# 34j/vr180-convert

Hardware: NVIDIA B200
Metric: SBS equirect output Mpix/s (higher is better)
Workload: dtype f64 coordinates / u8 fixed-point (INTER_BITS=5) sampling

## Files before the change

vr180-convert_b200/csrc/tiled.cu:

```cuda
#include "tiled.cuh"

namespace vr180 {
namespace tiled {

struct TileGeom {
    int rsel;
    int bx0, ry0;
    int x0, y0;
};

template <class M, int NV, bool DYN, int FR, bool SPLIT = false, bool VPAIR = false>
__device__ __forceinline__ void frame_loop(const RemapArgs& a, const TmaMaps& tm, int v_begin, int f0, int f1,
                                           const typename M::Pixel (&pc)[M::kPx], const TileGeom& tg, const int pitch,
                                           uint8_t* smem, int band, int cg, const DynRadius& dr,
                                           const double (&nx)[M::kPx], const double (&ny)[M::kPx], const short* tab) {
    static_assert(FR == 1 || !DYN, "a per-frame radius gives every frame its own rectangle");
    static_assert(M::kOutTiles / FR >= 2, "at least two out buffers of one item each");
    constexpr int kOutTileBytes = M::kTileH * kTileW * 3;
    constexpr int kOutItemBytes = FR * kOutTileBytes;
    constexpr int OB = M::kOutTiles / FR < kOutBufs ? M::kOutTiles / FR : kOutBufs;
    const int tid = threadIdx.x, lane = tid & 31, warp = tid >> 5;
    uint32_t s_stage = smem_u32(smem);
    asm volatile("" : "+r"(s_stage));
    const uint32_t s_full = s_stage + Lay<M>::kOffBar;
    const uint32_t s_ofull = s_full + 2 * kMaxStages * 8, s_oempty = s_ofull + kOutBufs * 8, s_out = s_stage + Lay<M>::kOffOut;

    int2* const s_org = reinterpret_cast<int2*>(smem + Lay<M>::kOffOrg);
    static_assert(!VPAIR || (SPLIT && FR == 2 && NV == 2 && !DYN), "an eye pair is two one-frame boxes of two views");
    const int n_items = VPAIR ? (f1 - f0) : ((f1 - f0 + FR - 1) / FR) * NV;
    const int rect_bytes = (M::kRowsMin + tg.rsel * kRowsStep) * pitch;
    const int stage_bytes = FR * rect_bytes;
    const int frame_pitch = SPLIT ? (rect_bytes + 127) & ~127 : rect_bytes;
    const int stage_stride = (FR * frame_pitch + 127) & ~127;
    static_assert(Lay<M>::kStageArea % 128 == 0 && Lay<M>::kStageArea / 128 <= 1024, "float quotient below");
    const int S = min(kMaxStages, (int)__fdividef((float)(Lay<M>::kStageArea / 128) + 0.5f, (float)(stage_stride >> 7)));

    if (warp == kSamplers / 32) {
        if (lane != 0) return;
        const CUtensorMap* const map0 = &tm.src[v_begin][(pitch - kPitchMin) / kPitchStep][tg.rsel];
        const int dst_x0 = (a.view[v_begin].dst_x_offset + tg.x0) * 3;
        const int dst_x1 = (a.view[v_begin + NV - 1].dst_x_offset + tg.x0) * 3;
        int p_item = 0, p_stage = 0;
        auto load = [&]() {
            const uint32_t bar = s_full + p_stage * 8;
            const int v = (NV == 2 && !VPAIR) ? (p_item & 1) : 0;
            const int f = VPAIR ? f0 + p_item : f0 + FR * ((NV == 2) ? (p_item >> 1) : p_item);
            int bx0 = tg.bx0, ry0 = tg.ry0;
            if (DYN) {
                const double rad = __ldg(dr.radius + f);
                if (rad == rad) {
                    int xlo, xhi, ylo, yhi;
                    dyn_range<M>(dr.ext[0], dr.ext[1], rad, dr.cx, xlo, xhi);
                    dyn_range<M>(dr.ext[2], dr.ext[3], rad, dr.cy, ylo, yhi);
                    const TileRect rc = tile_rect<M>(xlo, xhi, ylo, yhi);
                    bx0 = rc.bx0;
                    ry0 = rc.ry0;
                } else {
                    bx0 = ry0 = -(1 << 20);
                }
                s_org[p_stage] = make_int2(bx0, ry0);
            }
            mbar_expect_tx(bar, (uint32_t)stage_bytes);
            if (SPLIT) {
#pragma unroll
                for (int fr = 0; fr < FR; ++fr)
                    tma_load_3d(s_stage + p_stage * stage_stride + fr * frame_pitch,
                                map0 + (VPAIR ? fr : v) * (kWidths * kRowSizes), bx0, ry0, VPAIR ? f : f + fr, bar);
            } else {
                tma_load_3d(s_stage + p_stage * stage_stride, map0 + v * (kWidths * kRowSizes), bx0, ry0, f, bar);
            }
            ++p_item;
            if (++p_stage == S) p_stage = 0;
        };
        for (int n = 0; n < S && n < n_items; ++n) load();
        for (int n = 0; n < n_items; ++n) {
            const int o = n & (OB - 1);
            const int v = (NV == 2 && !VPAIR) ? (n & 1) : 0;
            const int f = VPAIR ? f0 + n : f0 + FR * ((NV == 2) ? (n >> 1) : n);
            mbar_wait(s_ofull + o * 8, (uint32_t)(n / OB) & 1u);
            if (n + S < n_items) load();
            if (SPLIT) {
#pragma unroll
                for (int fr = 0; fr < FR; ++fr)
                    tma_store_3d(&tm.dst, (VPAIR ? fr : v) ? dst_x1 : dst_x0, tg.y0, VPAIR ? f : f + fr,
                                 s_out + o * kOutItemBytes + fr * kOutTileBytes);
            } else {
                tma_store_3d(&tm.dst, v ? dst_x1 : dst_x0, tg.y0, f, s_out + o * kOutItemBytes);
            }
            bulk_commit();
            bulk_wait_read<0>();
            mbar_arrive(s_oempty + o * 8);
        }
        bulk_wait_read<0>();
        return;
    }

    const int sub = lane & 3;
    const uint32_t out_sel = sub == 0 ? 0x4210u : (sub == 1 ? 0x5421u : 0x6542u);
    const bool writer = sub != 3;
    constexpr int kOutStep = M::kRowPatch ? kTileW * 3 : 24;
    const int sw = band * (4 / M::kPx) + cg;
    uint32_t outp = s_out + (M::kRowPatch ? (M::kPx * sw) * (kTileW * 3) + (3 * (lane >> 2) + sub) * 4
                                          : (4 * band + (lane >> 3)) * (kTileW * 3) + M::kPx * cg * 24 +
                                                (3 * ((lane & 7) >> 2) + sub) * 4);
    uint32_t flags = (writer ? 1u : 0u) | (lane == 0 ? 2u : 0u);
    asm volatile("" : "+r"(outp), "+r"(flags));

    int st = 0;
    uint32_t ph = 0;
    typename M::Pixel cur[M::kPx];
    double cur_rad = CUDART_NAN;
    bool cur_have = false;
#pragma unroll
    for (int k = 0; k < M::kPx; ++k) cur[k] = pc[k];
    for (int n = 0; n < n_items; ++n) {
        mbar_wait(s_full + st * 8, ph);
        const uint32_t buf = s_stage + st * stage_stride;
        uint32_t res[FR][M::kPx];
        if (DYN) {
            const int f = f0 + ((NV == 2) ? (n >> 1) : n);
            const double rad = __ldg(dr.radius + f);
            if (!(rad == cur_rad)) {
                const int2 org = s_org[st];
                cur_have = rad == rad;
#pragma unroll
                for (int k = 0; k < M::kPx; ++k) {
                    const int qx = denorm_q<M>(nx[k], rad, dr.cx), qy = denorm_q<M>(ny[k], rad, dr.cy);
                    const int off = ((qy >> M::kShift) - M::kLo - org.y) * pitch + 3 * ((qx >> M::kShift) - M::kLo) - org.x;
                    M::set_offset(cur[k], off, cur_have);
                    M::weights(cur[k], qx & 31, qy & 31, tab);
                }
                cur_rad = rad;
            }
#pragma unroll
            for (int k = 0; k < M::kPx; ++k) {
                const uint32_t r = M::sample(buf, cur[k], (uint32_t)pitch);
                res[0][k] = cur_have ? r : 0u;
            }
        }
        uint32_t word[FR][M::kPx];
        if (!DYN && M::kInterp == VR180_INTER_LANCZOS4) {
#pragma unroll
            for (int k = 0; k < M::kPx; ++k) {
                uint32_t r[FR];
                sample_item<M, FR>(buf, (uint32_t)frame_pitch, pc[k], (uint32_t)pitch, r);
#pragma unroll
                for (int fr = 0; fr < FR; ++fr) res[fr][k] = r[fr];
            }
        }
#pragma unroll
        for (int fr = 0; fr < FR; ++fr) {
            if (!DYN && M::kInterp != VR180_INTER_LANCZOS4) {
#pragma unroll
                for (int k = 0; k < M::kPx; ++k) res[fr][k] = M::sample(buf + fr * frame_pitch, pc[k], (uint32_t)pitch);
            }
#pragma unroll
            for (int k = 0; k < M::kPx; ++k)
                word[fr][k] = __byte_perm(res[fr][k], __shfl_down_sync(0xffffffffu, res[fr][k], 1), out_sel);
        }
        const int o = n & (OB - 1);
        if (n >= OB) mbar_wait(s_oempty + o * 8, (uint32_t)(n / OB + 1) & 1u);
        if (flags & 1u) {
            const uint32_t ob = outp + o * kOutItemBytes;
#pragma unroll
            for (int fr = 0; fr < FR; ++fr)
#pragma unroll
                for (int k = 0; k < M::kPx; ++k) sts32(ob + fr * kOutTileBytes + k * kOutStep, word[fr][k]);
        }
        fence_proxy_async();
        __syncwarp();
        if (flags & 2u) mbar_arrive(s_ofull + o * 8);
        if (++st == S) { st = 0; ph ^= 1u; }
    }
}

template <class M, bool DYN, int FR>
__global__ void __launch_bounds__(kThreads, 4)
k_warp_tiled(const __grid_constant__ RemapArgs a, const __grid_constant__ vr180_chain_t chain0,
             const __grid_constant__ vr180_chain_t chain1, const __grid_constant__ TiledParams tp,
             const __grid_constant__ TmaMaps tm) {
    constexpr int kPx = M::kPx;
    constexpr int kChainUnroll = (FR == 1 && !DYN) ? kPx : 1;
    constexpr int kWarpsPerBand = 4 / kPx;
    extern __shared__ __align__(1024) uint8_t smem[];
    double* s_trig = reinterpret_cast<double*>(smem + Lay<M>::kOffTrig);
    int4* s_red = reinterpret_cast<int4*>(smem + Lay<M>::kOffRed);

    const int tid = threadIdx.x, lane = tid & 31, warp = tid >> 5;
    if (tid < 2 * kMaxStages + 2 * kOutBufs) {
        const uint32_t bars = smem_u32(smem + Lay<M>::kOffBar);
        const bool by_warps = (tid >= kMaxStages && tid < 2 * kMaxStages + kOutBufs);
        mbar_init(bars + tid * 8, by_warps ? kSamplers / 32 : 1);
        asm volatile("fence.mbarrier_init.release.cluster;" ::: "memory");
    }
    int* const s_cost = reinterpret_cast<int*>(smem + Lay<M>::kOffCost);
    if (tid < kPitchCands) s_cost[tid] = 0;
    const int tx = blockIdx.x, ty = blockIdx.y, tile = ty * tp.tiles_x + tx;
    const int x0 = tx * kTileW, y0 = ty * M::kTileH;
    const bool two_groups = !a.share_map && a.n_views == 2;
    const int g = two_groups ? (int)(blockIdx.z & 1u) : 0;
    const int chunk = two_groups ? (int)(blockIdx.z >> 1) : (int)blockIdx.z;
    const ViewArgs& mv = a.view[g];
    const int v_begin = g, v_end = a.share_map ? a.n_views : g + 1, nv = v_end - v_begin;
    const int f0 = chunk * a.frames_per_cta, f1 = min(a.n_frames, f0 + a.frames_per_cta);
    const bool sampler = warp < kSamplers / 32;
    const int sw = warp & (kSamplers / 32 - 1), band = sw / kWarpsPerBand, cg = sw % kWarpsPerBand;
    const int lx = M::kRowPatch ? lane : 8 * kPx * cg + (lane & 7), ly = M::kRowPatch ? kPx * sw : 4 * band + (lane >> 3);
    auto pcol = [&](int k) { return M::kRowPatch ? lx : lx + 8 * k; };
    auto prow = [&](int k) { return M::kRowPatch ? ly + k : ly; };
    const bool full_tile = (x0 + kTileW <= a.W) && (y0 + M::kTileH <= a.H);

    TileHdr hdr = {0, 0, 0, 0, 0};
    if (mv.map_kind != VR180_MAPSRC_ANALYTIC && mv.packed) hdr = decode_header(packed_header_raw(mv.packed, tile));
    const bool packed_tile = (hdr.flags & 1) != 0;

    int sx[kPx], sy[kPx];
    double nx[kPx], ny[kPx];
#pragma unroll
    for (int k = 0; k < kPx; ++k) {
        sx[k] = sy[k] = 0;
        nx[k] = ny[k] = 0.0;
    }
    constexpr bool dyn = DYN;
    if (mv.map_kind == VR180_MAPSRC_ANALYTIC) {
        const vr180_chain_t& ch = mv.chain_idx ? chain1 : chain0;
        const StdChain& sc = tp.std[mv.chain_idx ? 1 : 0];
        const bool fastc = sc.valid && sc.fast && !(tp.debug & 256);
        if (sc.valid || tp.sep_prefix) {
            if (tid < 64) {
                const bool is_row = tid >= 32;
                const int idx = tid & 31;
                const double* nm = ch.ops[0].p;
                const double c = (double)((is_row ? y0 : x0) + idx);
                const double n = mul_rn(__ddiv_rn(add_rn(c, -(is_row ? nm[1] : nm[0])), nm[2]), 2.0);
                double sv, cv;
                sincos(mul_rn(n, kHalfPi), &sv, &cv);
                if (fastc) {
                    std_tables(sc.R, sc.lat_is_y != 0, is_row, sv, cv, s_trig, s_trig + 128, idx);
                } else {
                    s_trig[(is_row ? 64 : 0) + idx] = sv;
                    s_trig[(is_row ? 96 : 32) + idx] = cv;
                }
            }
            __syncthreads();
            const bool lat_is_y = ch.ops[1].iparam != 0;
            auto seed = [&](int k, ChainState& s) {
                const double s_row = s_trig[64 + prow(k)], c_row = s_trig[96 + prow(k)];
                const double s_col = s_trig[pcol(k)], c_col = s_trig[32 + pcol(k)];
                s.mode = MODE_VEC3;
                s.x = s.y = s.r = s.ux = s.uy = 0.0;
                if (lat_is_y) {
                    s.vx = mul_rn(c_row, s_col);
                    s.vy = s_row;
                    s.vz = mul_rn(c_row, c_col);
                } else {
                    s.vx = s_col;
                    s.vy = mul_rn(c_col, s_row);
                    s.vz = mul_rn(c_col, c_row);
                }
            };
            if (!sampler) {
            } else if (fastc) {
                auto std_eval = [&](const StdChain& c) {
                    const bool x_fixed = M::kRowPatch ? !c.lat_is_y : (c.lat_is_y != 0);
                    const int fi = M::kRowPatch ? lx : ly;
                    const double* const ft = s_trig + (x_fixed ? 0 : 128) + fi;
                    const double f0 = ft[0], f1 = ft[32], f2 = ft[64], f3 = x_fixed ? ft[96] : 0.0;
#pragma unroll(kChainUnroll)
                    for (int k = 0; k < kPx; ++k) {
                        const int vi = M::kRowPatch ? prow(k) : pcol(k);
                        double vx, vy, vz;
                        if (x_fixed) {
                            vx = fma(f0, s_trig[128 + vi], f1); vy = fma(f0, s_trig[160 + vi], f2); vz = fma(f0, s_trig[192 + vi], f3);
                        } else {
                            const double sc_ = s_trig[vi];
                            vx = fma(sc_, f0, s_trig[32 + vi]); vy = fma(sc_, f1, s_trig[64 + vi]); vz = fma(sc_, f2, s_trig[96 + vi]);
                        }
                        double ox, oy;
                        int qx = 0, qy = 0;
                        if (dyn) {
                            std_pixel<true>(vx, vy, vz, c.poly, c.n_poly, c.den, ox, oy);
                        } else {
                            std_pixel<false>(vx, vy, vz, c.poly, c.n_poly, c.den, ox, oy);
                            qx = M::quant(__double2float_rn(ox));
                            qy = M::quant(__double2float_rn(oy));
                        }
#pragma unroll
                        for (int kk = 0; kk < kPx; ++kk)
                            if (kk == k) { sx[kk] = qx; sy[kk] = qy; nx[kk] = ox; ny[kk] = oy; }
                    }
                };
                if (mv.chain_idx) std_eval(tp.std[1]);
                else std_eval(tp.std[0]);
            } else {
#pragma unroll 1
                for (int k = 0; k < kPx; ++k) {
                    ChainState s;
                    seed(k, s);
                    run_ops(ch, 2, ch.n_ops - (dyn ? 1 : 0), s);
                    to_xy(s);
                    const int qx = M::quant(__double2float_rn(s.x)), qy = M::quant(__double2float_rn(s.y));
#pragma unroll
                    for (int kk = 0; kk < kPx; ++kk)
                        if (kk == k) { sx[kk] = qx; sy[kk] = qy; nx[kk] = s.x; ny[kk] = s.y; }
                }
            }
        } else if (sampler) {
#pragma unroll 1
            for (int k = 0; k < kPx; ++k) {
                double xs, ys;
                if (dyn) eval_chain_normalised(ch, x0 + pcol(k), y0 + prow(k), xs, ys);
                else eval_chain(ch, x0 + pcol(k), y0 + prow(k), xs, ys);
                const int qx = M::quant(__double2float_rn(xs)), qy = M::quant(__double2float_rn(ys));
#pragma unroll
                for (int kk = 0; kk < kPx; ++kk)
                    if (kk == k) { sx[kk] = qx; sy[kk] = qy; nx[kk] = xs; ny[kk] = ys; }
            }
        }
    } else if (sampler) {
        bool unpacked = false;
// ... 14 lines not shown
        for (int k = 0; k < kPx; ++k) {
            if (unpacked) break;
            const int i = x0 + pcol(k), j = y0 + prow(k);
            sx[k] = sy[k] = (int)0x80000000;
            if (i < a.W && j < a.H) {
                if (mv.map_kind == VR180_MAPSRC_FLOAT2) {
                    sx[k] = M::quant(__ldg(mv.xmap + (long long)j * mv.map_pitch + i));
                    sy[k] = M::quant(__ldg(mv.ymap + (long long)j * mv.map_pitch + i));
                } else {
                    const int2 q = __ldg(mv.fixed + (long long)j * mv.map_pitch + i);
                    sx[k] = q.x;
                    sy[k] = q.y;
                }
            }
        }
    }

    bool dynr = dyn;
    if (dyn) {
        const vr180_chain_t& ch = mv.chain_idx ? chain1 : chain0;
        const double r0 = __ldg(mv.radius_dev + f0);
        int same = r0 == r0;
        for (int f = f0 + 1 + lane; f < f1; f += 32) same &= __ldg(mv.radius_dev + f) == r0;
        if (__all_sync(0xffffffffu, same)) {
            dynr = false;
            const double cx = ch.ops[ch.n_ops - 1].p[2], cy = ch.ops[ch.n_ops - 1].p[3];
#pragma unroll
            for (int k = 0; k < kPx; ++k) {
                sx[k] = denorm_q<M>(nx[k], r0, cx);
                sy[k] = denorm_q<M>(ny[k], r0, cy);
            }
        }
    }

    if (!packed_tile) block_box_store<M>(sx, sy, s_red, warp, lane == 0 && sampler);
    DynRadius dr;
    dr.radius = nullptr;
    dr.cx = dr.cy = 0.0;
    dr.ext[0] = dr.ext[1] = dr.ext[2] = dr.ext[3] = 0.0;
    int nan_px = 0;
    if (dynr) {
        double* s_ext = reinterpret_cast<double*>(smem + Lay<M>::kOffExt);
        double e0 = CUDART_INF, e1 = -CUDART_INF, e2 = CUDART_INF, e3 = -CUDART_INF;
        if (sampler) {
#pragma unroll
            for (int k = 0; k < kPx; ++k) {
                nan_px |= (nx[k] != nx[k]) | (ny[k] != ny[k]);
                e0 = fmin(e0, nx[k]);
                e1 = fmax(e1, nx[k]);
                e2 = fmin(e2, ny[k]);
                e3 = fmax(e3, ny[k]);
            }
        }
#pragma unroll
        for (int d = 16; d > 0; d >>= 1) {
            e0 = fmin(e0, __shfl_xor_sync(0xffffffffu, e0, d));
            e1 = fmax(e1, __shfl_xor_sync(0xffffffffu, e1, d));
            e2 = fmin(e2, __shfl_xor_sync(0xffffffffu, e2, d));
            e3 = fmax(e3, __shfl_xor_sync(0xffffffffu, e3, d));
        }
        if (lane == 0 && sampler) {
            s_ext[warp * 4 + 0] = e0;
            s_ext[warp * 4 + 1] = e1;
            s_ext[warp * 4 + 2] = e2;
            s_ext[warp * 4 + 3] = e3;
        }
    }
    nan_px = __syncthreads_or(nan_px);
    static_assert(Lay<M>::kOffRed % 16 == 0, "s_red is read as int4");
    const int4 box = packed_tile ? make_int4(hdr.mnx, hdr.mxx, hdr.mny, hdr.mxy) : block_box_load(s_red, lane);
    const int mnx = box.x, mxx = box.y, mny = box.z, mxy = box.w;
    const TileRect rc = tile_rect<M>(mnx, mxx, mny, mxy);
    const bool vpair = !DYN && FR == 1 && nv == 2;
    const int fr_item = dynr ? 1 : (vpair ? 2 : FR);
    auto stage_fits = [&](int box_rows, int pitch_bytes) {
        const int rect = box_rows * pitch_bytes;
        return ((fr_item * ((DYN || vpair) ? (rect + 127) & ~127 : rect) + 127) & ~127) <= Lay<M>::kStageArea;
    };
    const int src_cols = a.view[v_begin].cols, src_rows = a.view[v_begin].rows;
    auto inside_src = [&](int x_lo, int x_hi, int y_lo, int y_hi) {
        return x_lo - M::kLo >= 0 && x_hi + M::kHi <= src_cols - 1 && y_lo - M::kLo >= 0 && y_hi + M::kHi <= src_rows - 1;
    };
    bool fast = full_tile && rc.wbytes <= kPitchMax && rc.rsel < kRowSizes && mnx > -32768 && mny > -32768 &&
                mxx < 32767 && mxy < 32767 && stage_fits(rc.box_rows, max(rc.wbytes, kPitchMin)) &&
                (tp.zero_border || inside_src(mnx, mxx, mny, mxy));
    int dyn_wbytes = 0, dyn_nrows = 0;
    if (dynr) {
        const double* s_ext = reinterpret_cast<const double*>(smem + Lay<M>::kOffExt);
        dr.ext[0] = dr.ext[2] = CUDART_INF;
        dr.ext[1] = dr.ext[3] = -CUDART_INF;
#pragma unroll
        for (int w = 0; w < kSamplers / 32; ++w) {
            dr.ext[0] = fmin(dr.ext[0], s_ext[w * 4 + 0]);
            dr.ext[1] = fmax(dr.ext[1], s_ext[w * 4 + 1]);
            dr.ext[2] = fmin(dr.ext[2], s_ext[w * 4 + 2]);
            dr.ext[3] = fmax(dr.ext[3], s_ext[w * 4 + 3]);
        }
        const vr180_chain_t& ch = mv.chain_idx ? chain1 : chain0;
        dr.radius = mv.radius_dev;
        dr.cx = ch.ops[ch.n_ops - 1].p[2];
        dr.cy = ch.ops[ch.n_ops - 1].p[3];
        int ok = 1;
        for (int f = f0 + lane; f < f1; f += 32) {
            const double rad = __ldg(dr.radius + f);
            if (rad == rad) {
                int lo, hi, ylo, yhi;
                dyn_range<M>(dr.ext[0], dr.ext[1], rad, dr.cx, lo, hi);
                ok &= (lo > -32768) & (hi < 32767);
                dyn_range<M>(dr.ext[2], dr.ext[3], rad, dr.cy, ylo, yhi);
                ok &= (ylo > -32768) & (yhi < 32767);
                const TileRect rf = tile_rect<M>(lo, hi, ylo, yhi);
                dyn_wbytes = max(dyn_wbytes, rf.wbytes);
                dyn_nrows = max(dyn_nrows, rf.nrows);
                if (!tp.zero_border) ok &= inside_src(lo, hi, ylo, yhi) ? 1 : 0;
            } else if (!tp.zero_border) {
                ok = 0;
            }
        }
        dyn_wbytes = __reduce_max_sync(0xffffffffu, dyn_wbytes);
        dyn_nrows = __reduce_max_sync(0xffffffffu, dyn_nrows);
        ok = __all_sync(0xffffffffu, ok);
        fast = full_tile && ok && !nan_px && dyn_wbytes <= kPitchMax && box_rsel<M>(dyn_nrows) < kRowSizes &&
               stage_fits(M::kRowsMin + box_rsel<M>(dyn_nrows) * kRowsStep, max(dyn_wbytes, kPitchMin));
    }

    if (!fast) {
        if (sampler) {
#pragma unroll
            for (int k = 0; k < kPx; ++k) {
                const int i = x0 + pcol(k), j = y0 + prow(k);
                if (i < a.W && j < a.H) {
                    for (int f = f0; f < f1; ++f) {
                        int qx = sx[k], qy = sy[k];
                        if (dynr) {
                            const double rad = __ldg(dr.radius + f);
                            qx = denorm_q<M>(nx[k], rad, dr.cx);
                            qy = denorm_q<M>(ny[k], rad, dr.cy);
                        }
                        gather_pixel<M>(a, f, i, j, v_begin, v_end, qx, qy, tp.tab);
                    }
                }
            }
        }
        return;
    }

    int pitch = max(dynr ? dyn_wbytes : rc.wbytes, kPitchMin);
    if (!dynr && (f1 - f0) * nv >= 8) {
        if (sampler) pitch_costs<M>(sx[0], sy[0], rc, pitch, lane, s_cost);
        __syncthreads();
        pitch = pick_pitch(s_cost, pitch, rc.box_rows, [&](int pe) { return stage_fits(rc.box_rows, pe); });
    }

    typename M::Pixel pc[kPx];
#pragma unroll
    for (int k = 0; k < kPx; ++k) {
        const int ix = sx[k] >> M::kShift, iy = sy[k] >> M::kShift;
        const int off = (iy - M::kLo - rc.ry0) * pitch + 3 * (ix - M::kLo) - rc.bx0;
        M::set_offset(pc[k], off, true);
        if (sampler && !dynr) M::weights(pc[k], sx[k] & 31, sy[k] & 31, tp.tab);
    }
    if constexpr (M::kWeightSmem != 0) {
        if (!dynr && sampler) {
            uint8_t* slot = smem + Lay<M>::kOffW + tid * 16;
#pragma unroll
            for (int ky = 0; ky < 8; ++ky)
                *reinterpret_cast<uint4*>(slot + ky * (kSamplers * 16)) = __ldg(reinterpret_cast<const uint4*>(pc[0].w) + ky);
            pc[0].ws = smem_u32(slot);
        }
    }
    TileGeom tg;
    tg.rsel = dynr ? box_rsel<M>(dyn_nrows) : rc.rsel;
    tg.bx0 = rc.bx0;
    tg.ry0 = rc.ry0;
    tg.x0 = x0;
    tg.y0 = y0;
    if (DYN && dynr) {
        if (nv == 2) frame_loop<M, 2, DYN, 1>(a, tm, v_begin, f0, f1, pc, tg, pitch, smem, band, cg, dr, nx, ny, tp.tab);
        else         frame_loop<M, 1, DYN, 1>(a, tm, v_begin, f0, f1, pc, tg, pitch, smem, band, cg, dr, nx, ny, tp.tab);
    } else {
        if constexpr (!DYN && FR == 1) {
            if (nv == 2) frame_loop<M, 2, false, 2, true, true>(a, tm, v_begin, f0, f1, pc, tg, pitch, smem, band, cg, dr, nx, ny, tp.tab);
            else         frame_loop<M, 1, false, 1, false>(a, tm, v_begin, f0, f1, pc, tg, pitch, smem, band, cg, dr, nx, ny, tp.tab);
        } else {
            if (nv == 2) frame_loop<M, 2, false, FR, DYN>(a, tm, v_begin, f0, f1, pc, tg, pitch, smem, band, cg, dr, nx, ny, tp.tab);
            else         frame_loop<M, 1, false, FR, DYN>(a, tm, v_begin, f0, f1, pc, tg, pitch, smem, band, cg, dr, nx, ny, tp.tab);
        }
    }
}

template <class M>
__global__ void __launch_bounds__(kSamplers) k_pack_tiles(const float* __restrict__ xmap, const float* __restrict__ ymap,
                                                         long long map_pitch, int W, int H, int tiles_x, int n_tiles,
                                                         void* __restrict__ packed) {
    constexpr int kPx = M::kPx;
    __shared__ int4 s_red[kSamplers / 32];
    __shared__ int s_cost[kPitchCands];
    const int tid = threadIdx.x, lane = tid & 31, sw = tid >> 5;
    const int tx = blockIdx.x % tiles_x, ty = blockIdx.x / tiles_x;
    const int x0 = tx * kTileW, y0 = ty * M::kTileH;
    const bool full_tile = (x0 + kTileW <= W) && (y0 + M::kTileH <= H);
    if (tid < kPitchCands) s_cost[tid] = 0;
    int sx[kPx], sy[kPx];
#pragma unroll
    for (int k = 0; k < kPx; ++k) {
        const int i = x0 + lane, j = y0 + kPx * sw + k;
        sx[k] = sy[k] = (int)0x80000000;
        if (i < W && j < H) {
            sx[k] = M::quant(__ldg(xmap + (long long)j * map_pitch + i));
            sy[k] = M::quant(__ldg(ymap + (long long)j * map_pitch + i));
        }
    }
    block_box_store<M>(sx, sy, s_red, sw, lane == 0);
    __syncthreads();
    const int4 box = block_box_load(s_red, lane);
    const int mnx = box.x, mxx = box.y, mny = box.z, mxy = box.w;
    const bool ok = full_tile && mnx > -32768 && mny > -32768 && mxx < 32767 && mxy < 32767 && mxx - mnx <= 255 &&
                    mxy - mny <= 255;
    const TileRect rc = tile_rect<M>(mnx, mxx, mny, mxy);
    const bool stageable = ok && rc.wbytes <= kPitchMax && rc.rsel < kRowSizes;
    const int pitch0 = max(rc.wbytes, kPitchMin);
    if (stageable) pitch_costs<M>(sx[0], sy[0], rc, pitch0, lane, s_cost);
    __syncthreads();
    const int pitch = !stageable ? kPitchMin : pick_pitch(s_cost, pitch0, rc.box_rows, [&](int pe) {
        return pe == pitch0 || rc.box_rows * pe <= kStreamSlotBytes<M>;
    });
    const int widx = (pitch - kPitchMin) / kPitchStep;
    if (tid == 0) {
        int4 h;
        h.x = (mnx & 0xffff) | (mxx << 16);
        h.y = (mny & 0xffff) | (mxy << 16);
        h.z = (ok ? kHdrPackable : 0) | (stageable ? kHdrStageable : 0) |
              (stageable && rc.box_rows * pitch <= kStreamSlotBytes<M> ? kHdrFitsSlot : 0) | (widx << 8) | (rc.rsel << 12);
        h.w = 0;
        reinterpret_cast<int4*>(packed)[blockIdx.x] = h;
    }
    uint32_t* ent = reinterpret_cast<uint32_t*>(static_cast<uint8_t*>(packed) + packed_entries_offset(n_tiles)) +
                    ((size_t)blockIdx.x * kSamplers + tid) * kPx;
#pragma unroll
    for (int k = 0; k < kPx; ++k) {
        const int ix = sat16(sx[k] >> M::kShift), iy = sat16(sy[k] >> M::kShift);
        const uint32_t fx = M::kShift ? (uint32_t)(sx[k] & 31) : 0u, fy = M::kShift ? (uint32_t)(sy[k] & 31) : 0u;
        ent[k] = ok ? ((uint32_t)(ix - mnx) | ((uint32_t)(iy - mny) << 8) | (fx << 16) | (fy << 21)) : 0u;
    }
}

}

static int tile_height_of(int interp) {
    return interp == VR180_INTER_LINEAR || interp == VR180_INTER_NEAREST ? tiled::LinearP::kTileH
           : interp == VR180_INTER_CUBIC                                  ? tiled::Cubic::kTileH
           : interp == VR180_INTER_LANCZOS4                               ? tiled::Lanczos4::kTileH
                                                                          : 0;
}

size_t packed_lut_bytes(int out_w, int out_h, int interp) {
    const int th = tile_height_of(interp);
    if (!th) return 0;
    const long long n_tiles = (long long)((out_w + tiled::kTileW - 1) / tiled::kTileW) * ((out_h + th - 1) / th);
    return tiled::packed_entries_offset(n_tiles) + (size_t)n_tiles * tiled::kTileW * th * 4;
}

int launch_pack_lut_tiles(const float* xmap, const float* ymap, int64_t map_pitch, int W, int H, int interp, void* packed,
                          cudaStream_t st) {
    using namespace tiled;
    const int th = tile_height_of(interp);
    if (!th) return VR180_ERR_UNSUPPORTED;
    const int tiles_x = (W + kTileW - 1) / kTileW, tiles_y = (H + th - 1) / th;
    const long long n_tiles = (long long)tiles_x * tiles_y;
    if (n_tiles > 0x7fffffffLL) return VR180_ERR_UNSUPPORTED;
    const dim3 grid((unsigned)n_tiles);
    if (interp == VR180_INTER_NEAREST)
        k_pack_tiles<Nearest><<<grid, kSamplers, 0, st>>>(xmap, ymap, (long long)map_pitch, W, H, tiles_x, (int)n_tiles, packed);
    else if (interp == VR180_INTER_LINEAR)
        k_pack_tiles<LinearP><<<grid, kSamplers, 0, st>>>(xmap, ymap, (long long)map_pitch, W, H, tiles_x, (int)n_tiles, packed);
    else if (interp == VR180_INTER_CUBIC)
        k_pack_tiles<Cubic><<<grid, kSamplers, 0, st>>>(xmap, ymap, (long long)map_pitch, W, H, tiles_x, (int)n_tiles, packed);
    else
        k_pack_tiles<Lanczos4><<<grid, kSamplers, 0, st>>>(xmap, ymap, (long long)map_pitch, W, H, tiles_x, (int)n_tiles, packed);
    g_launches.fetch_add(1, std::memory_order_relaxed);
    VR180_CUDA(cudaGetLastError());
    return VR180_OK;
}

static void match_std_chain(const vr180_chain_t& c, tiled::StdChain& out) {
    memset(&out, 0, sizeof(out));
    out.n_poly = -1;
    if (c.n_ops < 4 || c.ops[0].code != VR180_OP_NORMALIZE || c.ops[1].code != VR180_OP_EQUIRECT_ENC) return;
    memcpy(out.norm, c.ops[0].p, sizeof(out.norm));
    out.lat_is_y = c.ops[1].iparam != 0;
    int k = 2;
    if (c.ops[k].code == VR180_OP_ROT3) {
        out.has_rot = 1;
        memcpy(out.R, c.ops[k].p, sizeof(out.R));
        ++k;
    }
    if (k < c.n_ops && c.ops[k].code == VR180_OP_POLY) {
        out.n_poly = c.ops[k].iparam;
        memcpy(out.poly, c.ops[k].p, sizeof(out.poly));
        ++k;
    }
    if (k + 2 != c.n_ops || c.ops[k].code != VR180_OP_FISHEYE_DEC || c.ops[k].iparam != VR180_MAP_EQUIDISTANT ||
        c.ops[k + 1].code != VR180_OP_DENORMALIZE)
        return;
    memcpy(out.den, c.ops[k + 1].p, sizeof(out.den));
    out.valid = 1;
    if (!out.has_rot) {
        out.R[0] = out.R[4] = out.R[8] = 1.0;
        out.fast = 1;
    } else {
        double err = 0.0;
        for (int i = 0; i < 3; ++i)
            for (int j = 0; j < 3; ++j) {
                double d = i == j ? -1.0 : 0.0;
                for (int m = 0; m < 3; ++m) d += out.R[3 * m + i] * out.R[3 * m + j];
                err = std::fmax(err, std::fabs(d));
            }
        out.fast = err < 1e-12 ? 1 : 0;
    }
}

using EncodeTiledFn = CUresult (*)(CUtensorMap*, CUtensorMapDataType, cuuint32_t, void*, const cuuint64_t*,
                                   const cuuint64_t*, const cuuint32_t*, const cuuint32_t*, CUtensorMapInterleave,
                                   CUtensorMapSwizzle, CUtensorMapL2promotion, CUtensorMapFloatOOBfill);

static EncodeTiledFn encode_tiled_fn() {
    static EncodeTiledFn fn = [] {
        void* p = nullptr;
        cudaDriverEntryPointQueryResult q = cudaDriverEntryPointSymbolNotFound;
// ... 214 lines not shown
```

vr180-convert_b200/csrc/tiled.cuh:

```cuda
#pragma once
#include <cuda.h>

#include <cmath>
#include <cstdlib>
#include <mutex>
#include <type_traits>
#include <vector>

#include "chain_fast.cuh"
#include "common.cuh"
#include "sampler.cuh"

namespace vr180 {
namespace tiled {

constexpr int kTileW = 32;
constexpr int kSamplers = 256;
constexpr int kThreads = kSamplers + 32;
constexpr int kMaxStages = 8;
constexpr int kRowsStep = 4, kRowSizes = 9;
constexpr int kPitchMin = 96, kPitchMax = 256, kPitchStep = 16;
constexpr int kWidths = (kPitchMax - kPitchMin) / kPitchStep + 1;
constexpr int kPitchCands = 4;
constexpr int kStageAreaDefault = 40960;
// ... 240 lines not shown
        for (int ky = 0; ky < 4; ++ky, r += pitch / 4) {
            const uint32_t a0 = r[0], a1 = r[1], a2 = r[2], a3 = r[3];
            const uint32_t A0 = __funnelshift_r(a0, a1, sh), A1 = __funnelshift_r(a1, a2, sh),
                           A2 = __funnelshift_r(a2, a3, sh);
            const uint32_t q0 = __byte_perm(__byte_perm(A0, A1, 0x0630), A2, 0x5210);
            const uint32_t q1 = __byte_perm(__byte_perm(A0, A1, 0x0741), A2, 0x6210);
            const uint32_t q2 = __byte_perm(__byte_perm(A0, A1, 0x0052), A2, 0x7410);
            const uint32_t w01 = p.w[2 * ky], w23 = p.w[2 * ky + 1];
            acc0 = dp2a_hi_su(w23, q0, dp2a_lo_su(w01, q0, acc0));
            acc1 = dp2a_hi_su(w23, q1, dp2a_lo_su(w01, q1, acc1));
            acc2 = dp2a_hi_su(w23, q2, dp2a_lo_su(w01, q2, acc2));
        }
        return pack_sat_u8x3((int)acc0 >> 15, (int)acc1 >> 15, (int)acc2 >> 15);
    }
};

struct Lanczos4 {
    static constexpr int kPx = 1, kTileH = 8, kLo = 3, kHi = 4, kRowsMin = 16, kInterp = VR180_INTER_LANCZOS4;
    static constexpr bool kRowPatch = true;
    static constexpr int kShift = kInterBits;
    __device__ static __forceinline__ int quant(float m) { return quantise(m); }
    static constexpr int kStageArea = 16384, kWeightSmem = kSamplers * 128;
    static constexpr int kOutTiles = 4;
    struct Pixel {
        int boff;
        int sh;
        const short* w;
        uint32_t ws;
    };
    __device__ static __forceinline__ void set_offset(Pixel& p, int off, bool valid) {
        p.boff = valid ? (off & ~3) : 0;
        p.sh = (off & 3) * 8;
    }
    __device__ static __forceinline__ void weights(Pixel& p, int ax, int ay, const short* tab) {
        p.w = tab + (((ay << 5) | ax) << 6);
        p.ws = 0;
    }
    template <int NF>
    __device__ static __forceinline__ void sample_frames(uint32_t sbuf, uint32_t frame_bytes, const Pixel& p, uint32_t pitch,
                                                         uint32_t (&out)[NF]) {
        const uint8_t* base = static_cast<const uint8_t*>(__cvta_shared_to_generic(sbuf)) + p.boff;
        const int sh = p.sh;
        uint32_t acc[NF][3];
#pragma unroll
        for (int f = 0; f < NF; ++f) acc[f][0] = acc[f][1] = acc[f][2] = 16384u;
#pragma unroll
        for (int ky = 0; ky < 8; ++ky) {
            uint4 wv;
            if (p.ws) {
                asm volatile("ld.shared.v4.u32 {%0, %1, %2, %3}, [%4];"
                             : "=r"(wv.x), "=r"(wv.y), "=r"(wv.z), "=r"(wv.w)
                             : "r"(p.ws + ky * (kSamplers * 16)));
            } else {
                wv = __ldg(reinterpret_cast<const uint4*>(p.w + ky * 8));
            }
            const uint32_t wp[4] = {wv.x, wv.y, wv.z, wv.w};
#pragma unroll
            for (int f = 0; f < NF; ++f) {
                const uint32_t* r = reinterpret_cast<const uint32_t*>(base + f * frame_bytes + ky * pitch);
                uint32_t x[7], A[6];
#pragma unroll
                for (int i = 0; i < 7; ++i) x[i] = r[i];
#pragma unroll
                for (int i = 0; i < 6; ++i) A[i] = __funnelshift_r(x[i], x[i + 1], sh);
#pragma unroll
                for (int g = 0; g < 2; ++g) {
                    const uint32_t A0 = A[3 * g], A1 = A[3 * g + 1], A2 = A[3 * g + 2];
                    const uint32_t q0 = __byte_perm(__byte_perm(A0, A1, 0x0630), A2, 0x5210);
                    const uint32_t q1 = __byte_perm(__byte_perm(A0, A1, 0x0741), A2, 0x6210);
                    const uint32_t q2 = __byte_perm(__byte_perm(A0, A1, 0x0052), A2, 0x7410);
                    acc[f][0] = dp2a_hi_su(wp[2 * g + 1], q0, dp2a_lo_su(wp[2 * g], q0, acc[f][0]));
                    acc[f][1] = dp2a_hi_su(wp[2 * g + 1], q1, dp2a_lo_su(wp[2 * g], q1, acc[f][1]));
                    acc[f][2] = dp2a_hi_su(wp[2 * g + 1], q2, dp2a_lo_su(wp[2 * g], q2, acc[f][2]));
                }
            }
        }
#pragma unroll
        for (int f = 0; f < NF; ++f) {
            out[f] = pack_sat_u8x3((int)acc[f][0] >> 15, (int)acc[f][1] >> 15, (int)acc[f][2] >> 15);
        }
    }
    __device__ static __forceinline__ uint32_t sample(uint32_t sbuf, const Pixel& p, uint32_t pitch) {
        uint32_t out[1];
        sample_frames<1>(sbuf, 0u, p, pitch, out);
        return out[0];
    }
};

struct DynRadius {
    const double* radius;
    double cx, cy;
    double ext[4];
};
template <class M>
__device__ __forceinline__ int denorm_q(double n, double rad, double c) {
    return M::quant(__double2float_rn(add_rn(mul_rn(n, rad), c)));
}
template <class M>
__device__ __forceinline__ void dyn_range(double nmin, double nmax, double rad, double c, int& lo, int& hi) {
    const int a = sat16(denorm_q<M>(nmin, rad, c) >> M::kShift), b = sat16(denorm_q<M>(nmax, rad, c) >> M::kShift);
    lo = min(a, b);
    hi = max(a, b);
}

template <class M>
__device__ __forceinline__ void block_box_store(const int (&sx)[M::kPx], const int (&sy)[M::kPx], int4* s_red, int warp,
                                                bool store) {
    int mnx = INT_MAX, mxx = INT_MIN, mny = INT_MAX, mxy = INT_MIN;
#pragma unroll
    for (int k = 0; k < M::kPx; ++k) {
        const int ix = sat16(sx[k] >> M::kShift), iy = sat16(sy[k] >> M::kShift);
        mnx = min(mnx, ix);
        mxx = max(mxx, ix);
        mny = min(mny, iy);
        mxy = max(mxy, iy);
    }
    mnx = __reduce_min_sync(0xffffffffu, mnx);
    mxx = __reduce_max_sync(0xffffffffu, mxx);
    mny = __reduce_min_sync(0xffffffffu, mny);
    mxy = __reduce_max_sync(0xffffffffu, mxy);
    if (store) s_red[warp] = make_int4(mnx, mxx, mny, mxy);
}
__device__ __forceinline__ int4 block_box_load(const int4* s_red, int lane) {
    int4 r = make_int4(INT_MAX, INT_MIN, INT_MAX, INT_MIN);
    if (lane < kSamplers / 32) r = s_red[lane];
    r.x = __reduce_min_sync(0xffffffffu, r.x);
    r.y = __reduce_max_sync(0xffffffffu, r.y);
    r.z = __reduce_min_sync(0xffffffffu, r.z);
    r.w = __reduce_max_sync(0xffffffffu, r.w);
    return r;
}

template <class M>
__device__ __forceinline__ int box_rsel(int nrows) {
    return nrows <= M::kRowsMin ? 0 : (nrows - M::kRowsMin + kRowsStep - 1) / kRowsStep;
}
struct TileRect {
    int bx0, wbytes;
    int ry0, nrows;
    int rsel, box_rows;
};
template <class M>
__device__ __forceinline__ TileRect tile_rect(int mnx, int mxx, int mny, int mxy) {
    TileRect r;
    r.bx0 = (3 * (mnx - M::kLo)) & ~15;
    r.wbytes = ((3 * (mxx + M::kHi + 1) + 15) & ~15) - r.bx0;
    r.ry0 = mny - M::kLo;
    r.nrows = mxy + M::kHi + 1 - r.ry0;
    r.rsel = box_rsel<M>(r.nrows);
    r.box_rows = M::kRowsMin + r.rsel * kRowsStep;
    return r;
}

template <class M>
__device__ __forceinline__ void pitch_costs(int sx0, int sy0, const TileRect& rc, int pitch0, int lane, int* s_cost) {
    const int row = (sy0 >> M::kShift) - M::kLo - rc.ry0, col = 3 * ((sx0 >> M::kShift) - M::kLo) - rc.bx0;
    int cost = 0;
#pragma unroll
    for (int e = 0; e < kPitchCands; ++e) {
        const int w = (row * (pitch0 + kPitchStep * e) + col) >> 2;
        const unsigned same = __match_any_sync(0xffffffffu, w);
        const bool leader = (__ffs(same) - 1) == lane;
        const unsigned lm = __ballot_sync(0xffffffffu, leader);
        int deg = 0;
        if (leader) deg = __popc(__match_any_sync(lm, w & 31));
        deg = __reduce_max_sync(0xffffffffu, deg);
        if (lane == e) cost = deg;
    }
    constexpr int kStepsPerWarp = M::kTileH * kTileW / kSamplers;
    constexpr int kLoads = M::kInterp == VR180_INTER_NEAREST ? 2 : M::kInterp == VR180_INTER_LINEAR ? 6
                         : M::kInterp == VR180_INTER_CUBIC ? 16 : 56;
    if (lane < kPitchCands) atomicAdd(&s_cost[lane], cost * (kStepsPerWarp * kLoads));
}
template <class Fits>
__device__ __forceinline__ int pick_pitch(const int* s_cost, int pitch0, int box_rows, Fits fits) {
    int best = 0, best_cost = INT_MAX;
#pragma unroll
    for (int e = 0; e < kPitchCands; ++e) {
        const int pe = pitch0 + kPitchStep * e;
        const int c = s_cost[e] + box_rows * pe / 64;
        if (pe <= kPitchMax && fits(pe) && c < best_cost) { best_cost = c; best = e; }
    }
    return pitch0 + kPitchStep * best;
}

template <class M>
__device__ __forceinline__ void gather_pixel(const RemapArgs& a, int f, int i, int j, int v_begin, int v_end, int qx, int qy,
                                             const short* tab) {
    uint8_t* drow = a.dst + (long long)f * a.dst_frame_stride + (long long)j * a.dst_pitch;
    for (int v = v_begin; v < v_end; ++v) {
        const ViewArgs& vw = a.view[v];
        Src s{vw.src + (long long)f * vw.frame_stride, vw.rows, vw.cols, vw.pitch};
        int px[3];
        if (M::kInterp == VR180_INTER_NEAREST)
            fetch_tap<3>(s, sat16(qx), sat16(qy), a.border_mode, a.bv, px);
        else if (M::kInterp == VR180_INTER_LINEAR)
            sample_linear<3>(s, qx, qy, a.border_mode, a.bv, px);
        else if (M::kInterp == VR180_INTER_CUBIC)
            sample_tab<3, 4>(s, qx, qy, tab, a.border_mode, a.bv, px);
        else
            sample_tab<3, 8>(s, qx, qy, tab, a.border_mode, a.bv, px);
        uint8_t* o = drow + (long long)(vw.dst_x_offset + i) * 3;
        o[0] = (uint8_t)px[0];
        o[1] = (uint8_t)px[1];
        o[2] = (uint8_t)px[2];
    }
}

template <class M, int FR>
__device__ __forceinline__ void sample_item(uint32_t sbuf, uint32_t frame_bytes, const typename M::Pixel& p, uint32_t pitch,
                                            uint32_t (&out)[FR]) {
    if constexpr (M::kInterp == VR180_INTER_LANCZOS4) {
        M::template sample_frames<FR>(sbuf, frame_bytes, p, pitch, out);
    } else {
#pragma unroll
        for (int f = 0; f < FR; ++f) out[f] = M::sample(sbuf + f * frame_bytes, p, pitch);
    }
}

inline int zero_border(const RemapArgs& a) {
    return (a.border_mode == VR180_BORDER_CONSTANT && !(a.bv[0] | a.bv[1] | a.bv[2])) ? 1 : 0;
}
template <auto Kernel>
int max_dyn_smem_once(int bytes, int& dev) {
    static std::atomic<int> done[64];
    dev = 0;
    VR180_CUDA(cudaGetDevice(&dev));
    if (dev < 64 && !done[dev].load(std::memory_order_acquire)) {
        VR180_CUDA(cudaFuncSetAttribute(Kernel, cudaFuncAttributeMaxDynamicSharedMemorySize, bytes));
        done[dev].store(1, std::memory_order_release);
    }
    return VR180_OK;
}

}

const tiled::TmaMaps* tma_maps_for(const RemapArgs& a0, int interp, int rows_min, int tile_h, int fr);
int tiled_debug_flags();
int launch_remap_stream(const RemapArgs& a, int interp, const short* weight_tab, cudaStream_t st);
}
```

Before: 719,200.

## Permute per-lane pixel order to reduce shared-memory bank conflicts in linear sampling

For the linear sampler in the two-frame, non-dynamic path, each thread group may reassign which of its four pixels it samples at each step. A greedy pairwise-swap search, using match/ballot warp intrinsics, picks the assignment that minimises the estimated shared-memory wavefronts of the gather loads. The permutation is packed into flags and used to write each result word back to its original output row. It adds a one-time setup search per tile, gated by a minimum item count, and debug bits can disable or force it.

```diff
diff --git a/vr180-convert_b200/csrc/tiled.cu b/vr180-convert_b200/csrc/tiled.cu
--- a/vr180-convert_b200/csrc/tiled.cu
+++ b/vr180-convert_b200/csrc/tiled.cu
@@ -7,7 +7,12 @@
     int rsel;
     int bx0, ry0;
     int x0, y0;
+    uint32_t qrows;
 };
+
+template <class M, bool DYN, int FR, bool SPLIT>
+constexpr bool kQuadOrder = std::is_same<M, LinearP>::value && !DYN && FR == 2 && !SPLIT;
+constexpr int kQuadOrderMinItems = 16;
 
 template <class M, int NV, bool DYN, int FR, bool SPLIT = false, bool VPAIR = false>
 __device__ __forceinline__ void frame_loop(const RemapArgs& a, const TmaMaps& tm, int v_begin, int f0, int f1,
@@ -103,7 +108,7 @@
     uint32_t outp = s_out + (M::kRowPatch ? (M::kPx * sw) * (kTileW * 3) + (3 * (lane >> 2) + sub) * 4
                                           : (4 * band + (lane >> 3)) * (kTileW * 3) + M::kPx * cg * 24 +
                                                 (3 * ((lane & 7) >> 2) + sub) * 4);
-    uint32_t flags = (writer ? 1u : 0u) | (lane == 0 ? 2u : 0u);
+    uint32_t flags = (writer ? 1u : 0u) | (lane == 0 ? 2u : 0u) | (kQuadOrder<M, DYN, FR, SPLIT> ? tg.qrows << 8 : 0u);
     asm volatile("" : "+r"(outp), "+r"(flags));
 
     int st = 0;
@@ -165,7 +170,10 @@
 #pragma unroll
             for (int fr = 0; fr < FR; ++fr)
 #pragma unroll
-                for (int k = 0; k < M::kPx; ++k) sts32(ob + fr * kOutTileBytes + k * kOutStep, word[fr][k]);
+                for (int k = 0; k < M::kPx; ++k) {
+                    const uint32_t row = kQuadOrder<M, DYN, FR, SPLIT> ? (flags >> (8 + 4 * k)) & 3u : (uint32_t)k;
+                    sts32(ob + fr * kOutTileBytes + row * kOutStep, word[fr][k]);
+                }
         }
         fence_proxy_async();
         __syncwarp();
@@ -486,6 +494,33 @@
         pitch = pick_pitch(s_cost, pitch, rc.box_rows, [&](int pe) { return stage_fits(rc.box_rows, pe); });
     }
 
+    uint32_t qrows = 0x3210u;
+    if constexpr (kQuadOrder<M, DYN, FR, false>) {
+        if (sampler && !dynr && (f1 - f0) * nv >= kQuadOrderMinItems && !(tp.debug & 16)) {
+            if (tp.debug & 32) {
+                qrows = 0x0123u;
+            } else {
+                int w0[kPx];
+#pragma unroll
+                for (int k = 0; k < kPx; ++k)
+                    w0[k] = (((sy[k] >> M::kShift) - rc.ry0) * pitch + 3 * (sx[k] >> M::kShift) - rc.bx0) >> 2;
+                qrows = quad_order(w0, lane);
+            }
+            int px[kPx], py[kPx];
+#pragma unroll
+            for (int k = 0; k < kPx; ++k) {
+                const uint32_t r = (qrows >> (4 * k)) & 3u;
+                px[k] = r == 0 ? sx[0] : r == 1 ? sx[1] : r == 2 ? sx[2] : sx[3];
+                py[k] = r == 0 ? sy[0] : r == 1 ? sy[1] : r == 2 ? sy[2] : sy[3];
+            }
+#pragma unroll
+            for (int k = 0; k < kPx; ++k) {
+                sx[k] = px[k];
+                sy[k] = py[k];
+            }
+        }
+    }
+
     typename M::Pixel pc[kPx];
 #pragma unroll
     for (int k = 0; k < kPx; ++k) {
@@ -509,6 +544,7 @@
     tg.ry0 = rc.ry0;
     tg.x0 = x0;
     tg.y0 = y0;
+    tg.qrows = qrows;
     if (DYN && dynr) {
         if (nv == 2) frame_loop<M, 2, DYN, 1>(a, tm, v_begin, f0, f1, pc, tg, pitch, smem, band, cg, dr, nx, ny, tp.tab);
         else         frame_loop<M, 1, DYN, 1>(a, tm, v_begin, f0, f1, pc, tg, pitch, smem, band, cg, dr, nx, ny, tp.tab);
diff --git a/vr180-convert_b200/csrc/tiled.cuh b/vr180-convert_b200/csrc/tiled.cuh
--- a/vr180-convert_b200/csrc/tiled.cuh
+++ b/vr180-convert_b200/csrc/tiled.cuh
@@ -416,19 +416,22 @@
     return r;
 }
 
+__device__ __forceinline__ int lds_wavefronts(int w, int lane) {
+    const unsigned same = __match_any_sync(0xffffffffu, w);
+    const bool leader = (__ffs(same) - 1) == lane;
+    const unsigned lm = __ballot_sync(0xffffffffu, leader);
+    int deg = 0;
+    if (leader) deg = __popc(__match_any_sync(lm, w & 31));
+    return __reduce_max_sync(0xffffffffu, deg);
+}
+
 template <class M>
 __device__ __forceinline__ void pitch_costs(int sx0, int sy0, const TileRect& rc, int pitch0, int lane, int* s_cost) {
     const int row = (sy0 >> M::kShift) - M::kLo - rc.ry0, col = 3 * ((sx0 >> M::kShift) - M::kLo) - rc.bx0;
     int cost = 0;
 #pragma unroll
     for (int e = 0; e < kPitchCands; ++e) {
-        const int w = (row * (pitch0 + kPitchStep * e) + col) >> 2;
-        const unsigned same = __match_any_sync(0xffffffffu, w);
-        const bool leader = (__ffs(same) - 1) == lane;
-        const unsigned lm = __ballot_sync(0xffffffffu, leader);
-        int deg = 0;
-        if (leader) deg = __popc(__match_any_sync(lm, w & 31));
-        deg = __reduce_max_sync(0xffffffffu, deg);
+        const int deg = lds_wavefronts((row * (pitch0 + kPitchStep * e) + col) >> 2, lane);
         if (lane == e) cost = deg;
     }
     constexpr int kStepsPerWarp = M::kTileH * kTileW / kSamplers;
@@ -436,6 +439,40 @@
                          : M::kInterp == VR180_INTER_CUBIC ? 16 : 56;
     if (lane < kPitchCands) atomicAdd(&s_cost[lane], cost * (kStepsPerWarp * kLoads));
 }
+__device__ __forceinline__ uint32_t quad_order(const int (&w0)[4], int lane) {
+    int w[4], c[4];
+#pragma unroll
+    for (int k = 0; k < 4; ++k) {
+        w[k] = w0[k];
+        c[k] = lds_wavefronts(w[k], lane);
+    }
+    uint32_t order = 0x3210u;
+    const int grp = lane >> 2;
+#pragma unroll
+    for (int a = 0; a < 3; ++a) {
+#pragma unroll
+        for (int b = a + 1; b < 4; ++b) {
+#pragma unroll 1
+            for (int g = 0; g < 8; ++g) {
+                const bool mine = grp == g;
+                const int wa = mine ? w[b] : w[a], wb = mine ? w[a] : w[b];
+                const int ca = lds_wavefronts(wa, lane), cb = lds_wavefronts(wb, lane);
+                if (ca + cb < c[a] + c[b]) {
+                    c[a] = ca;
+                    c[b] = cb;
+                    if (mine) {
+                        w[a] = wa;
+                        w[b] = wb;
+                        const uint32_t ra = (order >> (4 * a)) & 15u, rb = (order >> (4 * b)) & 15u;
+                        order = (order & ~((15u << (4 * a)) | (15u << (4 * b)))) | (rb << (4 * a)) | (ra << (4 * b));
+                    }
+                }
+            }
+        }
+    }
+    return order;
+}
+
 template <class Fits>
 __device__ __forceinline__ int pick_pitch(const int* s_cost, int pitch0, int box_rows, Fits fits) {
     int best = 0, best_cost = INT_MAX;
```

After: 285,500 (median of 6 runs). 60.3% lower.
